# JJanai/back2future

Measured on AMD Instinct MI355X. Metric: frame-triplets/sec at 3x1024x1920, higher is better.
Workload: dtype f32; 1 GPU; BASELINE.json configs[4] per-GPU share: batch=16 synthetic 3x1024x1920 triplets per GPU, random-init pwc.lua weights (Ours-Hard shape), outputs flow + occ + est[3]; batch_per_gpu=16, global_batch=16, height=1024, width=1920, parallelism=dp1: independent triplets per rank, one RCCL weight broadcast at init, hip_graph=True

## Files before the change

### back2future_amd/csrc/b2f_api.hip

```cpp
#include "b2f_ctx.h"

#include <cmath>
#include <cstdio>
#include <cstdlib>

using namespace b2f;

static thread_local std::string g_err;
namespace b2f {
int api_fail(const std::string &m)
{
    g_err = m;
    return 1;
}
const std::string &api_error() { return g_err; }

ConvSeg cp8_seg(const float *ptr, int C, size_t hw)
{
    ConvSeg sgm;
    sgm.ptr = ptr;
    sgm.img_stride = (long)(hw * (size_t)((C + 7) / 8 * 8));
    sgm.chunk_stride = (long)(hw * 8);
    sgm.pix_stride = 8;
    sgm.nchunks = 0;
// ... 467 lines not shown
    const int head_id1 = find_conv(c, KIND_FEAT, 2, 2), head_id2 = find_conv(c, KIND_FEAT, 3, 1);
    const bool head_fused = c->bf16_direct >= 2 && P.h[2] >= 4 && P.w[2] >= 4 && head_id1 >= 0 && head_id2 >= 0 &&
                            c->packed[(size_t)head_id1].wino == 3 && c->packed[(size_t)head_id2].wino == 5;
    for (int l = 2; l <= 7; ++l) {
        const int hi = P.h[l - 1], wi = P.w[l - 1], ho = P.h[l], wo = P.w[l];
        const int Ci = (l == 2) ? kImgC : kFeat[l - 1], Co = kFeat[l];
        if (l == 2 && P.seq) {
            Scope sc(c, s, "conv_first_seq", cap);
            HIPCHK(launch_conv_first_seq(dev_in, in_kind, P.nimg, P.H, P.W, c->wpk_dev + c->first_w_off, c->wpk_dev + c->first_b_off,
                                         A + P.tmp, s));
        } else if (l == 2) {
            Scope sc(c, s, "conv_first", cap);
            HIPCHK(launch_conv_first((const float *)dev_in, unit, B, P.H, P.W, c->wpk_dev + c->first_w_off,
                                     c->wpk_dev + c->first_b_off, A + P.tmp, s));
        } else if (l == 3 && head_fused) {
            const ConvSeg in2f = cp8_seg(A + P.cs[2], Co, (size_t)ho * wo);
            CHK(run_conv(c, s, cap, find_conv(c, KIND_FEAT, l, 2), &in2f, P.nimg, ho, wo, 1, 1, A + P.cs[l]));
            continue;
        } else {
            const ConvSeg in1 = cp8_seg(A + P.cs[l - 1], Ci, (size_t)hi * wi);
            CHK(run_conv(c, s, cap, find_conv(c, KIND_FEAT, l, 1), &in1, P.nimg, hi, wi, 2, 1, A + P.tmp));
        }
        if (l == 2 && head_fused) {
            const PackedConv &p1 = c->packed[find_conv(c, KIND_FEAT, 2, 2)], &p2 = c->packed[find_conv(c, KIND_FEAT, 3, 1)];
            HeadLaunch hl;
            hl.in = A + P.tmp; hl.in_img_stride = (long)((size_t)ho * wo * 16); hl.in_chunk_stride = (long)((size_t)ho * wo * 8); hl.in_pix_stride = 8;
            hl.H1 = ho; hl.W1 = wo;
            hl.w1 = c->wpk_dev + p1.w_off; hl.b1 = c->wpk_dev + p1.b_off; hl.w2 = c->wpk_dev + p2.w_off; hl.b2 = c->wpk_dev + p2.b_off;
            hl.out = A + P.cs[2];
            hl.Ho = P.h[3]; hl.Wo = P.w[3]; hl.nimg = P.nimg;
            hl.out_img_stride = (long)((size_t)hl.Ho * hl.Wo * 32); hl.out_chunk_stride = (long)((size_t)hl.Ho * hl.Wo * 8); hl.out_pix_stride = 8;
            char hname[48];
            snprintf(hname, sizeof hname, c->profile_layers ? "convH16_16to32_%dx%d" : "conv_head16_bf16", ho, wo);
            Scope sc(c, s, hname, cap);
            HIPCHK(launch_conv_head16(hl, s));
            continue;
        }
        const ConvSeg in2 = cp8_seg(A + P.tmp, Co, (size_t)ho * wo);
        CHK(run_conv(c, s, cap, find_conv(c, KIND_FEAT, l, 2), &in2, P.nimg, ho, wo, 1, 1, A + P.cs[l]));
    }
    if (full) {
        Scope sc(c, s, "avgpool2", cap);
        const size_t img_f = (size_t)B * P.H * P.W * kImgC;
        for (int f = 0; f < 2; ++f) {
            const float *src = A + P.img + (size_t)(f == 0 ? 0 : 2) * img_f;
            for (int k = 2; k <= 5; ++k) {
                const int hk = P.H >> (k - 2), wk = P.W >> (k - 2);
                float *dst = A + P.ds[k] + (size_t)f * B * (hk / 2) * (wk / 2) * kImgC;
                HIPCHK(launch_avgpool2_nhwc(src, B, hk, wk, kImgC, dst, s));
                src = dst;
            }
        }
    }
    for (int l = 7; l >= 3; --l) {
        const int h = P.h[l], w = P.w[l], Cl = kFeat[l];
        const size_t hw = (size_t)h * w;
        CorrLaunch cl;
        cl.ref = A + P.cs[l] + (size_t)P.fo * hw * Cl;
        cl.nbr_fut = A + P.cs[l] + (size_t)2 * P.fo * hw * Cl;
        cl.nbr_past = A + P.cs[l];
        cl.img_stride = (long)(hw * Cl);
        cl.chunk_stride = (long)(hw * 8);
        cl.pix_stride = 8;
        cl.flow = (l < 7) ? A + P.U[l] : nullptr;
        cl.flow_b = (l < 7 && past) ? A + P.UB[l] : nullptr;
        cl.k = (float)(20.0 / std::pow(2.0, l - 1));
        cl.out = A + P.cv;
        cl.out_img_stride = (long)(hw * kCvRec);
        cl.out_chunk_stride = (long)(hw * 8);
        cl.out_pix_stride = 8;
        cl.B = B; cl.C = Cl; cl.h = h; cl.w = w;
        cl.variant = c->corr_variant;
        cl.ablate = c->corr_ablate;
        {
            char cname[48];
            snprintf(cname, sizeof cname, c->profile_layers ? "warp_costvol_%dx%d" : "warp_costvol", h, w);
            Scope sc(c, s, cname, cap);
            HIPCHK(launch_warp_costvol(cl, s));
        }
        float *occ_out = full ? O.t_occ[l] : (l == 3 ? O.occ : nullptr);
        float *occ_out2 = (!full && l == 3 && c->past_flow) ? O.est3 : nullptr;
        if (occ_out || occ_out2) {
            CHK(run_decoder(c, s, cap, P, KIND_OCC, l, A + P.logits));
            {
                Scope sc(c, s, "softmax_nearest4", cap);
                if (occ_out) HIPCHK(launch_softmax_nearest4_planar(A + P.logits, 8, B, h, w, occ_out, s));
                if (occ_out2) HIPCHK(launch_softmax_nearest4_planar(A + P.logits, 8, B, h, w, occ_out2, s));
            }
        }
        CHK(run_decoder(c, s, cap, P, KIND_FLOW, l, A + P.fs));
        if (past) CHK(run_decoder(c, s, cap, P, KIND_PAST, l, A + P.bfs));
        float *skip_f = full ? O.t_ufs[l] : (l == 3 ? (O.flow ? O.flow : A + P.flow_planar) : nullptr);
        {
            Scope sc(c, s, "upsample_flow2x", cap);
            float *u = (l > 3) ? A + P.U[l - 1] : A + P.u2;
            HIPCHK(launch_upsample_flow2x(A + P.fs, 8, B, h, w, u, s));
            if (skip_f) HIPCHK(launch_upsample_flow2x_planar(u, 2, B, 2 * h, 2 * w, skip_f, s));
            if (past) {
                float *ub = (l > 3) ? A + P.UB[l - 1] : A + P.d[1];
                HIPCHK(launch_upsample_flow2x(A + P.bfs, 8, B, h, w, ub, s));
                if (O.t_ubfs[l]) HIPCHK(launch_upsample_flow2x_planar(ub, 2, B, 2 * h, 2 * w, O.t_ubfs[l], s));
            }
        }
        if (full) {
            Scope sc(c, s, "warp_image", cap);
            const int k = l - 2;
            const int hk = 4 * h, wk = 4 * w;
            const size_t img_f = (size_t)B * hk * wk * kImgC;
            const float *im1 = (k == 1) ? A + P.img : A + P.ds[k];
            const float *im3 = (k == 1) ? A + P.img + 2 * img_f : A + P.ds[k] + img_f;
            const float kk = (float)(20.0 / std::pow(2.0, l - 3));
            const float *fl1 = (past && O.t_ubfs[l]) ? O.t_ubfs[l] : O.t_ufs[l];
            if (O.t_iw1[l]) HIPCHK(launch_warp_image_planar(im1, fl1, -kk, B, hk, wk, O.t_iw1[l], s));
            if (O.t_iw3[l]) HIPCHK(launch_warp_image_planar(im3, O.t_ufs[l], kk, B, hk, wk, O.t_iw3[l], s));
        }
    }
    if (!full && O.est3 && !c->past_flow && P.seq) {
        Scope sc(c, s, "warp_image_seq", cap);
        HIPCHK(launch_warp_input_seq(dev_in, in_kind, O.flow ? O.flow : A + P.flow_planar, -20.0f, B, P.H, P.W, O.est3, s));
    } else if (!full && O.est3 && !c->past_flow) {
        Scope sc(c, s, "warp_image", cap);
        HIPCHK(launch_warp_input_planar((const float *)dev_in, unit, 0, O.flow ? O.flow : A + P.flow_planar, -20.0f, B, P.H, P.W,
                                        O.est3, s));
    }
    return 0;
}

}
int b2f::find_conv_id(const b2f_ctx *c, int kind, int level, int idx) { return find_conv(c, kind, level, idx); }
int b2f::run_conv_layer(b2f_ctx *c, hipStream_t s, bool cap, int conv_id, const ConvSeg *segs, int nimg, int H, int W, int stride,
                        int leaky, float *out)
{
    if (conv_id < 0) return fail("b2f: layer not present in this model");
    return run_conv(c, s, cap, conv_id, segs, nimg, H, W, stride, leaky, out);
}
int b2f::ensure_arena(b2f_ctx *c, size_t floats) { return ensure_workspace_floats(c, floats); }
int b2f::check_shape(int B, int H, int W)
{
    if (B <= 0 || H <= 0 || W <= 0) return fail("b2f: non-positive shape");
    if (H % 64 || W % 64) return fail("b2f: H and W must be multiples of 64 (7 pyramid levels, back2future.lua:54-67)");
    return 0;
}
namespace {

bool parse_random(const char *name, bool *past, unsigned long long *seed, float *gain)
{
    if (strncmp(name, "random:", 7) != 0) return false;
    std::string s(name + 7);
    std::vector<std::string> parts;
    size_t pos = 0;
    while (true) {
        size_t q = s.find(':', pos);
        parts.push_back(s.substr(pos, q == std::string::npos ? q : q - pos));
        if (q == std::string::npos) break;
        pos = q + 1;
    }
    if (parts[0] == "hard") *past = false;
    else if (parts[0] == "soft") *past = true;
    else return false;
    *seed = 2;
    *gain = 1.f;
    if (parts.size() > 1 && !parts[1].empty()) *seed = strtoull(parts[1].c_str(), nullptr, 10);
    if (parts.size() > 2 && !parts[2].empty()) *gain = strtof(parts[2].c_str(), nullptr);
    return true;
}

bool ends_with(const std::string &s, const char *suf)
{
    const size_t n = strlen(suf);
// ... 106 lines not shown
        else if (path == "Ours-Soft-ft-KITTI") path = "models/RoamingImages_H_KITTI_S.t7";
        else if (path == "Ours-Soft-ft-Sintel") path = "models/RoamingImages_H_Sintel_S.t7";
        if (ends_with(path, ".t7")) {
            std::string err;
            if (!load_t7_ex(path, g, !(graph_opts && *graph_opts), flat, err)) return fail("b2f_init: " + err);
            past = g.past_flow;
        } else if (ends_with(path, ".b2fw")) {
            FILE *f = fopen(path.c_str(), "rb");
            if (!f) return fail("b2f_init: cannot open " + path);
            fseek(f, 0, SEEK_END);
            const long sz = ftell(f);
            fseek(f, 0, SEEK_SET);
            flat.resize((size_t)sz / 4);
            const size_t rd = fread(flat.data(), 4, flat.size(), f);
            fclose(f);
            if (rd != flat.size()) return fail("b2f_init: short read on " + path);
            GraphOpts gp = g, gn = g;
            gp.past_flow = true; gn.past_flow = false;
            if ((long long)flat.size() == param_count(gp)) past = true;
            else if ((long long)flat.size() == param_count(gn)) past = false;
            else return fail("b2f_init: " + path + " does not hold a parameter set of this graph (with or without past-flow decoders)");
        } else {
            return fail(std::string("b2f_init: unknown model '") + name + "'");
        }
    }
    b2f_ctx *c = new b2f_ctx();
    c->device = device;
    c->g = g;
    {
        auto env_int = [](const char *k, long long dflt) {
            const char *v = getenv(k);
            if (!v) return dflt;
            char *end = nullptr;
            const long long x = strtoll(v, &end, 10);
            return end == v ? 1ll : x;
        };
        c->wino4_min_pixels = (int)env_int("B2F_WINO4_MIN_PIXELS", c->wino4_min_pixels);
        c->wino_split_pixels = (int)env_int("B2F_WINO_SPLIT_PIXELS", c->wino_split_pixels);
        c->wino8 = (int)env_int("B2F_WINO8", c->wino8);
        c->adaptive_kernels = (int)env_int("B2F_ADAPTIVE_KERNELS", c->adaptive_kernels);
        c->corr_variant = (int)env_int("B2F_CORR_VARIANT", env_int("B2F_CORR_LAT", c->corr_variant));
        c->op_wino_split = (int)env_int("B2F_OP_WINO_SPLIT", c->op_wino_split);
        c->use_graph = (int)env_int("B2F_USE_GRAPH", c->use_graph);
        c->host_graph = (int)env_int("B2F_HOST_GRAPH", c->host_graph);
        c->profile = (int)env_int("B2F_PROFILE", c->profile);
        c->corr_ablate = (int)env_int("B2F_CORR_ABLATE", c->corr_ablate);
        c->profile_layers = (int)env_int("B2F_PROFILE_LAYERS", c->profile_layers);
        c->wino4_persistent = (int)env_int("B2F_WINO4_PERSISTENT", c->wino4_persistent);
        c->wino1d = (int)env_int("B2F_WINO1D", c->wino1d);
        c->wino6 = (int)env_int("B2F_WINO6", c->wino6);
        c->wino6_min_pixels = (int)env_int("B2F_WINO6_MIN_PIXELS", c->wino6_min_pixels);
        c->s2_loader = (int)env_int("B2F_S2_LOADER", c->s2_loader);
        c->s2_tile_groups = (int)env_int("B2F_S2_TILE_GROUPS", c->s2_tile_groups);
#if B2F_EXPERIMENTS
        c->wino4_split = (int)env_int("B2F_WINO4_SPLIT", c->wino4_split);
        c->wino4_hybrid = (int)env_int("B2F_WINO4_HYBRID", c->wino4_hybrid);
        c->wino2_split = (int)env_int("B2F_WINO2_SPLIT", c->wino2_split);
#endif
        if (!use_wino()) { c->bf16_conv = 0; c->bf16_direct = 0; }
        c->bf16_direct = (int)env_int("B2F_BF16_DIRECT", c->bf16_direct);
        c->bf16_conv = (int)env_int("B2F_BF16_CONV", c->bf16_conv);
        c->s2_tiles_per_block = (int)env_int("B2F_S2_TILES_PER_BLOCK", c->s2_tiles_per_block);
        c->host_subbatch_pixels = env_int("B2F_HOST_SUBBATCH_PIXELS", c->host_subbatch_pixels);
        c->host_threads = (int)env_int("B2F_HOST_THREADS", c->host_threads);
        c->host_u8 = (int)env_int("B2F_HOST_U8", c->host_u8);
        c->host_ramp = (int)env_int("B2F_HOST_RAMP", c->host_ramp);
#if !B2F_EXPERIMENTS
        if (c->corr_variant == 2 || c->corr_variant == 4 || c->corr_variant == 6 || c->corr_variant == 8) {
            fprintf(stderr, "b2f_init: B2F_CORR_VARIANT=%d is an experiment kernel (build with `python -m back2future_amd.build --experiments`): using the default\n", c->corr_variant);
            c->corr_variant = -1;
        }
        if (c->bf16_direct == 1) {
            fprintf(stderr, "b2f_init: B2F_BF16_DIRECT=1 is an experiment (build with `python -m back2future_amd.build --experiments`): using the default (2)\n");
            c->bf16_direct = 2;
        }
#endif
    }
    if (hipStreamCreateWithFlags(&c->stream, hipStreamDefault) != hipSuccess) {
        delete c;
        return fail("b2f_init: hipStreamCreate failed");
    }
    if (install_weights(c, flat.data(), (long long)flat.size(), past) != 0) {
        b2f_destroy(c);
        return 1;
    }
    *out = c;
    return 0;
}
B2F_CATCH("b2f_init_ex")

void b2f_destroy(b2f_ctx *c)
{
    if (!c) return;
    (void)hipSetDevice(c->device);
    if (c->stream) (void)hipStreamSynchronize(c->stream);
    drop_graphs(c);
    drop_gen_out(c);
    for (ProfEvent &pe : c->prof_pending) { (void)hipEventDestroy(pe.a); (void)hipEventDestroy(pe.b); }
    for (hipEvent_t e : c->ev_pool) (void)hipEventDestroy(e);
    for (HostSlot &hs : c->slot) {
        if (hs.dev) (void)hipFree(hs.dev);
        if (hs.pin) (void)hipHostFree(hs.pin);
        for (hipEvent_t e : {hs.ev_in, hs.ev_comp, hs.ev_out})
            if (e) (void)hipEventDestroy(e);
    }
    if (c->s_in) (void)hipStreamDestroy(c->s_in);
// ... 86 lines not shown
    }
    else if (!strcmp(key, "wino1d")) {
        HIPCHK(hipSetDevice(c->device));
        HIPCHK(hipDeviceSynchronize());
        drop_graphs(c);
        const bool had = c->wino1d != 0;
        c->wino1d = value;
        if (had != (value != 0)) CHK(b2f_commit_weights(c));
    }
    else if (!strcmp(key, "wino6") || !strcmp(key, "wino6_min_pixels")) {
        HIPCHK(hipSetDevice(c->device));
        HIPCHK(hipDeviceSynchronize());
        drop_graphs(c);
        if (key[5] == '_') c->wino6_min_pixels = value;
        else {
            const bool had = c->wino6 != 0;
            c->wino6 = value;
            if (had != (value != 0)) CHK(b2f_commit_weights(c));
        }
    }
#if !B2F_EXPERIMENTS
    else if (!strcmp(key, "wino2_split") || !strcmp(key, "wino4_split") || !strcmp(key, "wino4_hybrid")) {
        if (value != 0) return fail(std::string("b2f_set_option: ") + key + " selects an experiment kernel (tools/experiments/csrc): build with `python -m back2future_amd.build --experiments` and load libb2f_exp.so");
    }
#else
    else if (!strcmp(key, "wino2_split")) {
        HIPCHK(hipSetDevice(c->device));
        HIPCHK(hipDeviceSynchronize());
        drop_graphs(c);
        const bool had = c->wino2_split != 0;
        c->wino2_split = value;
        if (had != (value != 0)) CHK(b2f_commit_weights(c));
    }
    else if (!strcmp(key, "wino4_split") || !strcmp(key, "wino4_hybrid")) {
        HIPCHK(hipSetDevice(c->device));
        HIPCHK(hipDeviceSynchronize());
        drop_graphs(c);
        const bool had = c->wino4_split || c->wino4_hybrid;
        (key[6] == 's' ? c->wino4_split : c->wino4_hybrid) = value;
        if (had != (c->wino4_split || c->wino4_hybrid)) CHK(b2f_commit_weights(c));
    }
#endif
    else if (!strcmp(key, "s2_tiles_per_block") || !strcmp(key, "wino4_persistent")) {
        HIPCHK(hipSetDevice(c->device));
        HIPCHK(hipDeviceSynchronize());
        drop_graphs(c);
        (key[0] == 's' ? c->s2_tiles_per_block : c->wino4_persistent) = value;
    }
    else if (!strcmp(key, "s2_loader") || !strcmp(key, "s2_tile_groups")) {
        HIPCHK(hipSetDevice(c->device));
        HIPCHK(hipDeviceSynchronize());
        drop_graphs(c);
        (key[3] == 'l' ? c->s2_loader : c->s2_tile_groups) = value;
    }
    else if (!strcmp(key, "wino_split_pixels") || !strcmp(key, "wino8")) {
        HIPCHK(hipSetDevice(c->device));
        HIPCHK(hipDeviceSynchronize());
        drop_graphs(c);
        (key[4] == '8' ? c->wino8 : c->wino_split_pixels) = value;
    }
    else if (!strcmp(key, "wino4_min_pixels") || !strcmp(key, "adaptive_kernels")) {
        HIPCHK(hipSetDevice(c->device));
        HIPCHK(hipDeviceSynchronize());
        drop_graphs(c);
        (key[0] == 'w' ? c->wino4_min_pixels : c->adaptive_kernels) = value;
    } else if (!strcmp(key, "corr_variant") || !strcmp(key, "corr_ablate")) {
        HIPCHK(hipSetDevice(c->device));
        HIPCHK(hipDeviceSynchronize());
        drop_graphs(c);
        if (key[5] == 'v' && !B2F_EXPERIMENTS && (value == 2 || value == 4 || value == 6 || value == 8))
            return fail("b2f_set_option: corr_variant 2 / 4 / 6 / 8 are experiment kernels: build with `python -m back2future_amd.build --experiments`");
        (key[5] == 'v' ? c->corr_variant : c->corr_ablate) = value;
    } else if (!strcmp(key, "op_wino_split")) c->op_wino_split = value;
    else if (!strcmp(key, "host_subbatch_pixels")) c->host_subbatch_pixels = value > 0 ? value : (16ll << 20);
    else if (!strcmp(key, "host_threads")) c->host_threads = value;
    else if (!strcmp(key, "host_u8")) c->host_u8 = value;
    else if (!strcmp(key, "host_ramp")) c->host_ramp = value;
    else if (!strcmp(key, "debug_fail_next")) c->debug_fail_next = value;
    else return fail(std::string("b2f_set_option: unknown key ") + key);
    return 0;
}
B2F_CATCH("b2f_set_option")

int b2f_get_option(const b2f_ctx *c, const char *key, int *value) try
{
    if (!c || !key || !value) return fail("b2f_get_option: null argument");
    const std::string k(key);
    if (k == "use_graph") *value = c->use_graph;
    else if (k == "host_graph") *value = c->host_graph;
    else if (k == "profile") *value = c->profile;
    else if (k == "profile_layers") *value = c->profile_layers;
    else if (k == "s2_tiles_per_block") *value = c->s2_tiles_per_block;
    else if (k == "wino4_persistent") *value = c->wino4_persistent;
    else if (k == "experiments") *value = B2F_EXPERIMENTS;
    else if (k == "wino1d") *value = c->wino1d;
    else if (k == "wino6") *value = c->wino6;
    else if (k == "wino6_min_pixels") *value = c->wino6_min_pixels;
    else if (k == "s2_loader") *value = c->s2_loader;
    else if (k == "s2_tile_groups") *value = c->s2_tile_groups;
    else if (k == "wino4_split") *value = c->wino4_split;
    else if (k == "wino4_hybrid") *value = c->wino4_hybrid;
    else if (k == "wino2_split") *value = c->wino2_split;
    else if (k == "bf16_direct") *value = c->bf16_direct;
    else if (k == "bf16_conv") *value = c->bf16_conv;
    else if (k == "bf16_conv_min_pixels") *value = c->bf16_conv_min_pixels;
    else if (k == "wino4_min_pixels") *value = c->wino4_min_pixels;
    else if (k == "wino_split_pixels") *value = c->wino_split_pixels;
    else if (k == "wino8") *value = c->wino8;
    else if (k == "adaptive_kernels") *value = c->adaptive_kernels;
    else if (k == "corr_variant") *value = c->corr_variant;
    else if (k == "corr_ablate") *value = c->corr_ablate;
    else if (k == "op_wino_split") *value = c->op_wino_split;
    else if (k == "host_subbatch_pixels") *value = (int)std::min<long long>(c->host_subbatch_pixels, 0x7fffffff);
    else if (k == "host_threads") *value = c->host_threads;
    else if (k == "host_u8") *value = c->host_u8;
    else if (k == "host_ramp") *value = c->host_ramp;
    else if (k == "debug_fail_next") *value = c->debug_fail_next;
    else return fail("b2f_get_option: unknown key " + k);
    return 0;
}
B2F_CATCH("b2f_get_option")

int b2f_synchronize(b2f_ctx *c) try
{
    if (!c) return fail("b2f_synchronize: null context");
    HIPCHK(hipSetDevice(c->device));
    HIPCHK(hipStreamSynchronize(c->stream));
    return 0;
}
B2F_CATCH("b2f_synchronize")

int b2f_profile_reset(b2f_ctx *c) try
{
    if (!c) return fail("b2f_profile_reset: null context");
    CHK(prof_collect(c));
    std::fill(c->prof_ms.begin(), c->prof_ms.end(), 0.0);
    std::fill(c->prof_n.begin(), c->prof_n.end(), 0);
    return 0;
}
B2F_CATCH("b2f_profile_reset")

int b2f_profile_read(b2f_ctx *c, char *names, double *total_ms, long long *launches, int cap, int *n) try
{
    if (!c || !n) return fail("b2f_profile_read: null argument");
    CHK(prof_collect(c));
    const int cnt = std::min<int>(cap, (int)c->prof_names.size());
    for (int i = 0; i < cnt; ++i) {
        if (names) { strncpy(names + 32 * i, c->prof_names[i].c_str(), 31); names[32 * i + 31] = 0; }
        if (total_ms) total_ms[i] = c->prof_ms[i];
        if (launches) launches[i] = c->prof_n[i];
    }
    *n = cnt;
// ... 472 lines not shown
```

### back2future_amd/csrc/b2f_ctx.h

```cpp
#pragma once
#include "../../include/b2f.h"

#include <algorithm>
#include <atomic>
#include <condition_variable>
#include <cstring>
#include <exception>
#include <map>
#include <memory>
#include <mutex>
#include <string>
#include <thread>
#include <tuple>
#include <vector>

#include "b2f_host.h"
#include "b2f_internal.h"

namespace b2f {

int api_fail(const std::string &m);
const std::string &api_error();


// ... 189 lines not shown
            l.unlock();
            run_piece(j);
            l.lock();
            if (++done_ == pieces_->size()) cv_done_.notify_all();
        }
    }
    std::vector<std::thread> th_;
    std::mutex m_;
    std::condition_variable cv_, cv_done_;
    const std::vector<CopyJob> *pieces_ = nullptr;
    size_t next_ = 0, done_ = 0;
    bool stop_ = false;
};

}

struct b2f_ctx {
    int device = 0;
    bool past_flow = false;
    b2f::GraphOpts g;
    long long nparams = 0;
    hipStream_t stream = nullptr;
    std::vector<b2f::ConvDesc> lay;
    std::vector<b2f::PackedConv> packed;
    float *w_dev = nullptr;
    float *wpk_dev = nullptr;
    size_t wpk_floats = 0;
    size_t first_w_off = 0, first_b_off = 0;
    float *arena = nullptr;
    size_t arena_floats = 0;
    int wsB = 0, wsH = 0, wsW = 0;
    int use_graph = 0, profile = 0;
    int host_graph = 1;
    int wino8 = 1;
    int wino_split_pixels = 512;
    int wino4_min_pixels = 4096;
    int cur_batch = 0;
    int req_batch = 0;
    int adaptive_kernels = -1;
    int corr_ablate = 0;
    int corr_variant = -1;
    int op_wino_split = 0;
    int profile_layers = 0;
    int bf16_direct = 2;
    int bf16_conv_min_pixels = 65536;
    int bf16_conv = 1;
    int wino2_split = 0;
    int wino4_hybrid = 0;
    int wino4_split = 0;
    int wino6 = 1;
    int wino6_min_pixels = 16384;
    int wino1d = 0;
    int s2_tile_groups = 1;
    int s2_loader = 1;
    int wino4_persistent = 1;
    int s2_tiles_per_block = 0;
    long long host_subbatch_pixels = 16ll << 20;
    int host_threads = 0;
    int host_u8 = 1, host_ramp = 1;
    int debug_fail_next = 0;
    std::map<b2f::GraphKey, hipGraphExec_t> graphs;
    std::vector<float *> gen_out;
    int genB = 0, genH = 0, genW = 0;
    std::vector<std::string> prof_names;
    std::vector<double> prof_ms;
    std::vector<long long> prof_n;
    std::vector<b2f::ProfEvent> prof_pending;
    std::vector<hipEvent_t> ev_pool;
    hipStream_t s_in = nullptr, s_out = nullptr;
    b2f::HostSlot slot[2];
    std::unique_ptr<b2f::CopyPool> pool_in, pool_out;
    b2f::DevWork dwork;
};

#define HIPCHK(expr)                                                                         \
    do {                                                                                     \
        hipError_t e_ = (expr);                                                              \
        if (e_ != hipSuccess)                                                                \
            return b2f::api_fail(std::string(#expr) + ": " + hipGetErrorString(e_));          \
    } while (0)
#define B2F_CATCH(fn_)                                                                        \
    catch (const std::exception &e_) { return b2f::api_fail(std::string(fn_ ": ") + e_.what()); } \
    catch (...) { return b2f::api_fail(fn_ ": unknown exception"); }
#define CHK(expr)                         \
    do {                                  \
        int rc_ = (expr);                 \
        if (rc_ != 0) return rc_;         \
    } while (0)

namespace b2f {
int check_shape(int B, int H, int W);
void drop_graphs(b2f_ctx *c);
void drop_gen_out(b2f_ctx *c);
int forward_device(b2f_ctx *c, const void *dev_in, int in_kind, int B, int H, int W, float *dev_flow, float *dev_occ,
                   float *dev_est3, hipStream_t s, bool graph, bool seq = false);
int check_request(const FlowRequest &r);
int compute_flow_host(b2f_ctx *c, const FlowRequest &r);
int compute_flow_device(b2f_ctx *c, const FlowRequest &r, void *stream);
ConvSeg cp8_seg(const float *ptr, int C, size_t hw);
int find_conv_id(const b2f_ctx *c, int kind, int level, int idx);
int run_conv_layer(b2f_ctx *c, hipStream_t s, bool cap, int conv_id, const ConvSeg *segs, int nimg, int H, int W, int stride, int leaky,
                   float *out);
int ensure_arena(b2f_ctx *c, size_t floats);
int graph_forward(b2f_ctx *c, hipStream_t s, bool cap, const void *dev_in, int in_kind, int B, int H, int W, float *const *outs);
}
```

### back2future_amd/csrc/b2f_glue.hip

```cpp
#include "b2f_internal.h"

namespace b2f {

__global__ void pack_input_kernel(const float *in, int normalize, int B, int H, int W, float *img)
{
    const size_t hw = (size_t)H * W;
    const size_t i = (size_t)blockIdx.x * blockDim.x + threadIdx.x;
    if (i >= (size_t)B * hw) return;
    const size_t b = i / hw, p = i - b * hw;
#pragma unroll
    for (int f = 0; f < 3; ++f) {
        float v[3];
#pragma unroll
        for (int c = 0; c < 3; ++c) {
            float x = in[(b * 9 + f * 3 + c) * hw + p];
            if (normalize) x = color_normalize(x, c);
            v[c] = x;
        }
        float4 *o = reinterpret_cast<float4 *>(img + (((size_t)f * B + b) * hw + p) * kImgC);
        o[0] = make_float4(v[0], v[1], v[2], 0.f);
        o[1] = make_float4(0.f, 0.f, 0.f, 0.f);
    }
}

hipError_t launch_pack_input(const float *in, int normalize, int B, int H, int W, float *img, hipStream_t s)
{
    const size_t n = (size_t)B * H * W;
    hipLaunchKernelGGL(pack_input_kernel, dim3((unsigned)((n + 255) / 256)), dim3(256), 0, s, in, normalize, B, H, W, img);
    return hipGetLastError();
}


__global__ void warp_nhwc_kernel(const float *img, long img_stride, int pix_stride, int C, int ih, int iw,
                                 const float *grid, float k, int B, int gh, int gw, float *out,
                                 int out_pix_stride)
{
    const size_t total = (size_t)B * gh * gw * C;
    const size_t i = (size_t)blockIdx.x * blockDim.x + threadIdx.x;
    if (i >= total) return;
    const int c = (int)(i % C);
    size_t pix = i / C;
    const int x = (int)(pix % gw);
    const size_t row = pix / gw;
    const int y = (int)(row % gh);
    const int b = (int)(row / gh);
    const float2 g = *reinterpret_cast<const float2 *>(grid + pix * 2);
    int xl, yt;
    float wx, wy;
    bhwd_top_left(g.x * k + (float)x, iw, xl, wx);
    bhwd_top_left(g.y * k + (float)y, ih, yt, wy);
    const float *src = img + (size_t)b * img_stride + ((size_t)yt * iw + xl) * pix_stride + c;
    const bool x1 = xl + 1 <= iw - 1, y1 = yt + 1 <= ih - 1;
    const float tl = src[0];
    const float tr = x1 ? src[pix_stride] : 0.f;
    const float bl = y1 ? src[(size_t)iw * pix_stride] : 0.f;
    const float br = (x1 && y1) ? src[(size_t)(iw + 1) * pix_stride] : 0.f;
    out[pix * out_pix_stride + c] = wx * wy * tl + (1.f - wx) * wy * tr + wx * (1.f - wy) * bl + (1.f - wx) * (1.f - wy) * br;
}

hipError_t launch_warp_nhwc(const float *img, long img_stride, int pix_stride, int C, int ih, int iw,
                            const float *grid, float k, int B, int gh, int gw, float *out,
                            int out_pix_stride, hipStream_t s)
{
    const size_t n = (size_t)B * gh * gw * C;
    hipLaunchKernelGGL(warp_nhwc_kernel, dim3((unsigned)((n + 255) / 256)), dim3(256), 0, s, img, img_stride,
                       pix_stride, C, ih, iw, grid, k, B, gh, gw, out, out_pix_stride);
    return hipGetLastError();
}

__device__ __forceinline__ float2 bilerp2(const float *in, int ps, int h, int w, float rh, float rw, int y2, int x2)
{
    const float h1r = rh * (float)y2;
    const int h1 = (int)h1r;
    const int h1p = (h1 < h - 1) ? 1 : 0;
    const float h1l = h1r - (float)h1, h0l = 1.f - h1l;
    const float w1r = rw * (float)x2;
    const int w1 = (int)w1r;
    const int w1p = (w1 < w - 1) ? 1 : 0;
    const float w1l = w1r - (float)w1, w0l = 1.f - w1l;
    const float *p = in + ((size_t)h1 * w + w1) * ps;
    const float2 a = *reinterpret_cast<const float2 *>(p), b = *reinterpret_cast<const float2 *>(p + (size_t)w1p * ps);
    const float2 c = *reinterpret_cast<const float2 *>(p + (size_t)h1p * w * ps);
    const float2 d = *reinterpret_cast<const float2 *>(p + ((size_t)h1p * w + w1p) * ps);
    float2 o;
    o.x = h0l * (w0l * a.x + w1l * b.x) + h1l * (w0l * c.x + w1l * d.x);
    o.y = h0l * (w0l * a.y + w1l * b.y) + h1l * (w0l * c.y + w1l * d.y);
    return o;
}

__global__ __launch_bounds__(256) void upsample_flow2x_kernel(const float *in, int ps, int B, int h, int w, float *out, int planar)
{
    const int H2 = 2 * h, W2 = 2 * w;
    const int x0 = 4 * (int)(blockIdx.x * blockDim.x + threadIdx.x);
    const int y2 = (int)blockIdx.y, b = (int)blockIdx.z;
    if (x0 >= W2) return;
    const float rh = (H2 > 1) ? (float)(h - 1) / (float)(H2 - 1) : 0.f;
    const float rw = (W2 > 1) ? (float)(w - 1) / (float)(W2 - 1) : 0.f;
    const float *src = in + (size_t)b * h * w * ps;
    float2 o[4];
#pragma unroll
    for (int k = 0; k < 4; ++k) o[k] = bilerp2(src, ps, h, w, rh, rw, y2, min(x0 + k, W2 - 1));
    const size_t hw2 = (size_t)H2 * W2, row = (size_t)y2 * W2 + x0;
    if (planar) {
        float *o0 = out + ((size_t)b * 2) * hw2 + row, *o1 = o0 + hw2;
        if ((W2 & 3) == 0) {
            *reinterpret_cast<float4 *>(o0) = make_float4(o[0].x, o[1].x, o[2].x, o[3].x);
            *reinterpret_cast<float4 *>(o1) = make_float4(o[0].y, o[1].y, o[2].y, o[3].y);
        } else {
#pragma unroll
            for (int k = 0; k < 4; ++k)
                if (x0 + k < W2) { o0[k] = o[k].x; o1[k] = o[k].y; }
        }
    } else {
        float2 *op = reinterpret_cast<float2 *>(out) + (size_t)b * hw2 + row;
        if ((W2 & 3) == 0) {
            *reinterpret_cast<float4 *>(op) = make_float4(o[0].x, o[0].y, o[1].x, o[1].y);
            *reinterpret_cast<float4 *>(op + 2) = make_float4(o[2].x, o[2].y, o[3].x, o[3].y);
        } else {
#pragma unroll
            for (int k = 0; k < 4; ++k)
                if (x0 + k < W2) op[k] = o[k];
        }
    }
}

static hipError_t launch_upsample(const float *in, int in_pix_stride, int B, int h, int w, float *out, int planar, hipStream_t s)
{
    if (B <= 0 || h <= 0 || w <= 0) return hipSuccess;
    if (2 * h > 65535 || B > 65535) return hipErrorInvalidValue;
    const int groups = (2 * w + 3) / 4;
    hipLaunchKernelGGL(upsample_flow2x_kernel, dim3((unsigned)((groups + 255) / 256), (unsigned)(2 * h), (unsigned)B), dim3(256), 0, s, in,
                       in_pix_stride, B, h, w, out, planar);
    return hipGetLastError();
}
hipError_t launch_upsample_flow2x(const float *in, int in_pix_stride, int B, int h, int w, float *out, hipStream_t s)
{
    return launch_upsample(in, in_pix_stride, B, h, w, out, 0, s);
}
hipError_t launch_upsample_flow2x_planar(const float *in, int in_pix_stride, int B, int h, int w, float *out, hipStream_t s)
{
    return launch_upsample(in, in_pix_stride, B, h, w, out, 1, s);
}

__global__ __launch_bounds__(256) void softmax_nearest4_kernel(const float *logits, int ps, int B, int h, int w, float *out)
{
    const int H4 = 4 * h, W4 = 4 * w;
    const int x = (int)(blockIdx.x * blockDim.x + threadIdx.x);
    const int Y = (int)blockIdx.y, b = (int)blockIdx.z;
    if (x >= w) return;
    const float2 z = *reinterpret_cast<const float2 *>(logits + (((size_t)b * h + (Y >> 2)) * w + x) * ps);
    const float m = fmaxf(z.x, z.y);
    const float e0 = expf(z.x - m), e1 = expf(z.y - m);
    const float sum = e0 + e1;
    const float p0 = e0 / sum, p1 = e1 / sum;
    const size_t hw4 = (size_t)H4 * W4;
    float *o0 = out + ((size_t)b * 2) * hw4 + (size_t)Y * W4 + 4 * x;
    *reinterpret_cast<float4 *>(o0) = make_float4(p0, p0, p0, p0);
    *reinterpret_cast<float4 *>(o0 + hw4) = make_float4(p1, p1, p1, p1);
}

hipError_t launch_softmax_nearest4_planar(const float *logits, int in_pix_stride, int B, int h, int w, float *out, hipStream_t s)
{
    if (B <= 0 || h <= 0 || w <= 0) return hipSuccess;
    if (4 * h > 65535 || B > 65535) return hipErrorInvalidValue;
    hipLaunchKernelGGL(softmax_nearest4_kernel, dim3((unsigned)((w + 255) / 256), (unsigned)(4 * h), (unsigned)B), dim3(256), 0, s, logits,
                       in_pix_stride, B, h, w, out);
    return hipGetLastError();
}

__global__ void warp_image_planar_kernel(const float *img8, const float *flow, float k, int B, int H, int W, float *out)
{
    const size_t hw = (size_t)H * W;
    const size_t i = (size_t)blockIdx.x * blockDim.x + threadIdx.x;
    if (i >= (size_t)B * hw) return;
    const size_t b = i / hw, p = i - b * hw;
    const int y = (int)(p / W), x = (int)(p - (size_t)y * W);
    const float u = flow[(b * 2) * hw + p] * k, v = flow[(b * 2 + 1) * hw + p] * k;
    int xl, yt;
    float wx, wy;
    bhwd_top_left(u + (float)x, W, xl, wx);
    bhwd_top_left(v + (float)y, H, yt, wy);
    const float *src = img8 + (b * hw + (size_t)yt * W + xl) * kImgC;
    const bool x1 = xl + 1 <= W - 1, y1 = yt + 1 <= H - 1;
    const float4 z = make_float4(0.f, 0.f, 0.f, 0.f);
    const float4 tl = *reinterpret_cast<const float4 *>(src);
    const float4 tr = x1 ? *reinterpret_cast<const float4 *>(src + kImgC) : z;
    const float4 bl = y1 ? *reinterpret_cast<const float4 *>(src + (size_t)W * kImgC) : z;
    const float4 br = (x1 && y1) ? *reinterpret_cast<const float4 *>(src + (size_t)(W + 1) * kImgC) : z;
    const float w00 = wx * wy, w01 = (1.f - wx) * wy, w10 = wx * (1.f - wy), w11 = (1.f - wx) * (1.f - wy);
    out[(b * 3) * hw + p] = w00 * tl.x + w01 * tr.x + w10 * bl.x + w11 * br.x;
    out[(b * 3 + 1) * hw + p] = w00 * tl.y + w01 * tr.y + w10 * bl.y + w11 * br.y;
    out[(b * 3 + 2) * hw + p] = w00 * tl.z + w01 * tr.z + w10 * bl.z + w11 * br.z;
}

hipError_t launch_warp_image_planar(const float *img8, const float *flow_planar, float k, int B, int H, int W,
                                    float *out, hipStream_t s)
{
    const size_t n = (size_t)B * H * W;
    hipLaunchKernelGGL(warp_image_planar_kernel, dim3((unsigned)((n + 255) / 256)), dim3(256), 0, s, img8, flow_planar, k, B, H, W, out);
    return hipGetLastError();
}


__global__ __launch_bounds__(256) __attribute__((amdgpu_waves_per_eu(8, 8))) void conv_first_kernel(const float *in, int normalize, int B, int H, int W,
                                                         const float *wt , const float *bias ,
                                                         float *out )
{
// ... 140 lines not shown
                    const int pp = (ty + ky) * P + tx + kx;
                    const float4 lo = patch[c][0][pp], hi = patch[c][1][pp];
                    const float4 *wk = wsh + (c * 9 + ky * 3 + kx) * 4;
                    const float4 w0 = wk[0], w1 = wk[1], w2 = wk[2], w3 = wk[3];
                    a0 = fmaf(lo.x, w0.x, a0);  a1 = fmaf(lo.x, w0.y, a1);
                    a0 = fmaf(lo.y, w0.z, a0);  a1 = fmaf(lo.y, w0.w, a1);
                    a0 = fmaf(lo.z, w1.x, a0);  a1 = fmaf(lo.z, w1.y, a1);
                    a0 = fmaf(lo.w, w1.z, a0);  a1 = fmaf(lo.w, w1.w, a1);
                    a0 = fmaf(hi.x, w2.x, a0);  a1 = fmaf(hi.x, w2.y, a1);
                    a0 = fmaf(hi.y, w2.z, a0);  a1 = fmaf(hi.y, w2.w, a1);
                    a0 = fmaf(hi.z, w3.x, a0);  a1 = fmaf(hi.z, w3.y, a1);
                    a0 = fmaf(hi.w, w3.z, a0);  a1 = fmaf(hi.w, w3.w, a1);
                }
        }
    }
    const int oy = oy0 + ty, ox = ox0 + tx;
    if (oy >= H || ox >= W) return;
    if (leaky) { a0 = a0 > 0.f ? a0 : 0.2f * a0; a1 = a1 > 0.f ? a1 : 0.2f * a1; }
    float *op = out + (size_t)img * out_img_stride + ((size_t)oy * W + ox) * out_pix_stride;
    *reinterpret_cast<float2 *>(op) = make_float2(a0, a1);
}

hipError_t launch_conv_narrow2(const ConvLaunch &p, hipStream_t s)
{
    if (p.stride != 1 || p.cout != 2 || p.nseg != 1 || (p.seg[0].pix_stride & 3) || (p.out_pix_stride & 1)) return hipErrorInvalidValue;
    const int tiles = ((p.W + 15) / 16) * ((p.H + 15) / 16);
    if ((long)tiles * p.nimg <= 3L * device_cu_count() && p.seg[0].nchunks > 2)
        hipLaunchKernelGGL(conv_narrow2_kernel<4>, dim3((unsigned)(tiles * p.nimg)), dim3(256), 0, s, p.seg[0].ptr, p.seg[0].img_stride,
                           p.seg[0].chunk_stride, p.seg[0].pix_stride, p.seg[0].nchunks, p.H, p.W, p.wpk, p.bias, p.out,
                           p.out_img_stride, p.out_pix_stride, p.leaky);
    else
        hipLaunchKernelGGL(conv_narrow2_kernel<2>, dim3((unsigned)(tiles * p.nimg)), dim3(256), 0, s, p.seg[0].ptr, p.seg[0].img_stride,
                           p.seg[0].chunk_stride, p.seg[0].pix_stride, p.seg[0].nchunks, p.H, p.W, p.wpk, p.bias, p.out,
                           p.out_img_stride, p.out_pix_stride, p.leaky);
    return hipGetLastError();
}

size_t narrow2_wpk_floats(int cin_chunks) { return (size_t)cin_chunks * 9 * 8 * 2; }

void narrow2_pack_weights(const float *w, const float *b, int Ci, const int *cin_map, int cin_chunks, float *wpk, float *bpk)
{
    for (int c = 0; c < cin_chunks; ++c)
        for (int t = 0; t < 9; ++t)
            for (int j = 0; j < 8; ++j)
                for (int o = 0; o < 2; ++o) {
                    const int k = c * kCK + j;
                    const int ci = cin_map ? cin_map[k] : (k < Ci ? k : -1);
                    wpk[((c * 9 + t) * 8 + j) * 2 + o] = ci >= 0 ? w[((size_t)o * Ci + ci) * 9 + t] : 0.f;
                }
    bpk[0] = b[0];
    bpk[1] = b[1];
}

__global__ void warp_input_planar_kernel(const float *in, int normalize, int frame, const float *flow, float k, int B,
                                         int H, int W, float *out)
{
    const size_t hw = (size_t)H * W;
    const size_t i = (size_t)blockIdx.x * blockDim.x + threadIdx.x;
    if (i >= (size_t)B * hw) return;
    const size_t b = i / hw, p = i - b * hw;
    const int y = (int)(p / W), x = (int)(p - (size_t)y * W);
    const float u = flow[(b * 2) * hw + p] * k, v = flow[(b * 2 + 1) * hw + p] * k;
    int xl, yt;
    float wx, wy;
    bhwd_top_left(u + (float)x, W, xl, wx);
    bhwd_top_left(v + (float)y, H, yt, wy);
    const int dx = (xl + 1 <= W - 1) ? 1 : 0, dy = (yt + 1 <= H - 1) ? W : 0;
    const float w00 = wx * wy, w01 = (1.f - wx) * wy, w10 = wx * (1.f - wy), w11 = (1.f - wx) * (1.f - wy);
#pragma unroll
    for (int c = 0; c < 3; ++c) {
        const float *src = in + (b * 9 + (size_t)frame * 3 + c) * hw + (size_t)yt * W + xl;
        float tl = src[0], tr = src[dx], bl = src[dy], br = src[dy + dx];
        if (normalize) {
            tl = color_normalize(tl, c); tr = color_normalize(tr, c);
            bl = color_normalize(bl, c); br = color_normalize(br, c);
        }
        out[(b * 3 + c) * hw + p] = w00 * tl + w01 * tr + w10 * bl + w11 * br;
    }
}

hipError_t launch_warp_input_planar(const float *in, int normalize, int frame, const float *flow_planar, float k, int B,
                                    int H, int W, float *out, hipStream_t s)
{
    const size_t n = (size_t)B * H * W;
    hipLaunchKernelGGL(warp_input_planar_kernel, dim3((unsigned)((n + 255) / 256)), dim3(256), 0, s, in, normalize, frame,
                       flow_planar, k, B, H, W, out);
    return hipGetLastError();
}

__global__ void avgpool2_kernel(const float *in, int nimg, int H, int W, int C, float *out)
{
    const int Ho = H / 2, Wo = W / 2, C4 = C / 4;
    const size_t n = (size_t)nimg * Ho * Wo * C4;
    const size_t i = (size_t)blockIdx.x * blockDim.x + threadIdx.x;
    if (i >= n) return;
    const int c4 = (int)(i % C4);
    size_t pix = i / C4;
    const int X = (int)(pix % Wo);
    const size_t r = pix / Wo;
    const int Y = (int)(r % Ho);
    const size_t b = r / Ho;
    const float4 *s = reinterpret_cast<const float4 *>(in) + ((b * H + 2 * Y) * W + 2 * X) * C4 + c4;
    const float4 a = s[0], bb = s[C4], c = s[(size_t)W * C4], d = s[(size_t)(W + 1) * C4];
    float4 o;
    o.x = (a.x + bb.x + c.x + d.x) / 4.0f;
    o.y = (a.y + bb.y + c.y + d.y) / 4.0f;
    o.z = (a.z + bb.z + c.z + d.z) / 4.0f;
    o.w = (a.w + bb.w + c.w + d.w) / 4.0f;
    reinterpret_cast<float4 *>(out)[i] = o;
}

hipError_t launch_avgpool2_nhwc(const float *in, int nimg, int H, int W, int C, float *out, hipStream_t s)
{
    const size_t n = (size_t)nimg * (H / 2) * (W / 2) * (C / 4);
    hipLaunchKernelGGL(avgpool2_kernel, dim3((unsigned)((n + 255) / 256)), dim3(256), 0, s, in, nimg, H, W, C, out);
    return hipGetLastError();
}

__global__ void nhwc_to_planar_kernel(const float *in, int pix_stride, int C, int B, int h, int w, float *out)
{
    const size_t hw = (size_t)h * w;
    const size_t n = (size_t)B * C * hw;
    const size_t i = (size_t)blockIdx.x * blockDim.x + threadIdx.x;
    if (i >= n) return;
    const size_t p = i % hw;
    const size_t bc = i / hw;
    const int c = (int)(bc % C);
    const size_t b = bc / C;
    out[i] = in[(b * hw + p) * pix_stride + c];
}

hipError_t launch_nhwc_to_planar(const float *in, int pix_stride, int C, int B, int h, int w, float *out, hipStream_t s)
{
    const size_t n = (size_t)B * C * h * w;
    hipLaunchKernelGGL(nhwc_to_planar_kernel, dim3((unsigned)((n + 255) / 256)), dim3(256), 0, s, in, pix_stride, C, B, h, w, out);
    return hipGetLastError();
}

__global__ void cp8_to_planar_kernel(const float *in, int C, int B, int h, int w, float *out)
// ... 54 lines not shown
```

### back2future_amd/csrc/b2f_internal.h

```cpp
#pragma once
#include <hip/hip_runtime.h>
#ifndef B2F_EXPERIMENTS
#define B2F_EXPERIMENTS 0
#endif
#include <cstdint>

namespace b2f {

constexpr int kLevels = 7, kLst = 3, kWin = 9, kND = 2 * kWin * kWin;
constexpr int kFeat[8] = {0, 3, 16, 32, 64, 96, 128, 192};
constexpr int kDec[7] = {0, 128, 128, 96, 64, 32, 2};
constexpr int kCvRec = 168;
constexpr int kCvChunks = 21;
constexpr int kImgC = 8;
constexpr int kCK = 8;

struct ConvSeg {
    const float *ptr;
    long img_stride;
    long chunk_stride;
    int pix_stride;
    int nchunks;
};
struct ConvLaunch {
// ... 130 lines not shown
    int ablate = 0;
    int variant = -1;
};
inline int attr_slot()
{
    int dev = 0;
    if (hipGetDevice(&dev) != hipSuccess || dev < 0) dev = 0;
    return dev & 63;
}
inline int device_cu_count()
{
    static int n_cu_dev[64] = {0};
    int &n = n_cu_dev[attr_slot()];
    if (!n) {
        int dev = 0, v = 0;
        if (hipGetDevice(&dev) != hipSuccess || hipDeviceGetAttribute(&v, hipDeviceAttributeMultiprocessorCount, dev) != hipSuccess || v <= 0) v = 256;
        n = v < 8 ? 8 : v;
    }
    return n;
}
#ifdef __HIPCC__
__device__ __forceinline__ int xcd_remap(int bid, int nwg)
{
    const int q = nwg >> 3, r = nwg & 7;
    const int xcd = bid & 7, k = bid >> 3;
    return (xcd < r ? xcd * (q + 1) : r * (q + 1) + (xcd - r) * q) + k;
}
__device__ __forceinline__ void bhwd_top_left(float coord, int size, int &pt, float &wt)
{
    float c = coord;
    if (c < 0.f) c = 0.f;
    if (c > (float)(size - 1)) c = (float)(size - 1);
    const float fl = floorf(c);
    pt = (int)fl;
    wt = 1.f - (c - fl);
}
#endif

inline int cv_slot(int dir, int c) { return c < 80 ? dir * 80 + c : 160 + dir; }
hipError_t launch_warp_costvol(const CorrLaunch &p, hipStream_t s);
bool warp_costvol_unit_supported(const CorrLaunch &p);
hipError_t launch_warp_costvol_unit(const CorrLaunch &p, hipStream_t s);
hipError_t launch_warp_costvol_spec(const CorrLaunch &p, hipStream_t s);
hipError_t launch_warp_costvol_gw(const CorrLaunch &p, hipStream_t s);
hipError_t launch_costvol_generic(const float *ref, const float *frm, int B, int C, int h, int w,
                                  int win, int fwd, float *out, hipStream_t s);

hipError_t launch_pack_input(const float *in, int normalize, int B, int H, int W, float *img,
                             hipStream_t s);
hipError_t launch_conv_first(const float *in, int normalize, int B, int H, int W, const float *wt,
                             const float *bias, float *out, hipStream_t s);
hipError_t launch_warp_input_planar(const float *in, int normalize, int frame, const float *flow_planar,
                                    float k, int B, int H, int W, float *out, hipStream_t s);
hipError_t launch_conv_first_seq(const void *in, int in_kind, int T, int H, int W, const float *wt, const float *bias,
                                 float *out, hipStream_t s);
hipError_t launch_warp_input_seq(const void *in, int in_kind, const float *flow_planar, float k, int B, int H, int W,
                                 float *out, hipStream_t s);
hipError_t launch_warp_nhwc(const float *img, long img_stride, int pix_stride, int C, int ih,
                            int iw, const float *grid, float k, int B, int gh, int gw,
                            float *out, int out_pix_stride, hipStream_t s);
hipError_t launch_upsample_flow2x(const float *in, int in_pix_stride, int B, int h, int w, float *out,
                                  hipStream_t s);
hipError_t launch_upsample_flow2x_planar(const float *in, int in_pix_stride, int B, int h, int w,
                                         float *out, hipStream_t s);
hipError_t launch_softmax_nearest4_planar(const float *logits, int in_pix_stride, int B, int h, int w,
                                          float *out, hipStream_t s);
hipError_t launch_warp_image_planar(const float *img8, const float *flow_planar, float k, int B,
                                    int H, int W, float *out, hipStream_t s);
hipError_t launch_avgpool2_nhwc(const float *in, int nimg, int H, int W, int C, float *out,
                                hipStream_t s);
hipError_t launch_nhwc_to_planar(const float *in, int pix_stride, int C, int B, int h, int w,
                                 float *out, hipStream_t s);
hipError_t launch_cp8_to_planar(const float *in, int C, int B, int h, int w, float *out, hipStream_t s);
hipError_t launch_planar_to_nhwc(const float *in, int C, int B, int h, int w, float *out,
                                 int pix_stride, hipStream_t s);
hipError_t launch_fill(float *p, size_t n, float v, hipStream_t s);

hipError_t launch_image_scale(const float *src, int normalize, long planes, int Hs, int Ws, float *tmp, float *dst,
                              int Hd, int Wd, hipStream_t s);
hipError_t launch_outputs_f32(const float *flow_net, const float *occ, const float *est3, int est3_ch, int B, int fh, int fw, int H0,
                              int W0, double sc_w, double sc_h, float *flow, float *occ_prob, unsigned char *fwd_occ,
                              unsigned char *bwd_occ, hipStream_t s);
hipError_t launch_unpack_u8(const unsigned char *in, size_t n, float *out, hipStream_t s);

}
```

Measured before the change: 845.1 triplets/s.

## Fuse final flow upsampling, occlusion softmax and input warp into one kernel

```diff
diff --git a/back2future_amd/csrc/b2f_api.hip b/back2future_amd/csrc/b2f_api.hip
--- a/back2future_amd/csrc/b2f_api.hip
+++ b/back2future_amd/csrc/b2f_api.hip
@@ -543,6 +543,7 @@
             }
         }
     }
+    const bool fused_out = c->output_fused && !full && !c->past_flow && !P.seq && O.est3 && in_kind != B2F_IN_U8 && P.H == 4 * P.h[3] && P.W == 4 * P.w[3];
     for (int l = 7; l >= 3; --l) {
         const int h = P.h[l], w = P.w[l], Cl = kFeat[l];
         const size_t hw = (size_t)h * w;
@@ -569,11 +570,12 @@
             Scope sc(c, s, cname, cap);
             HIPCHK(launch_warp_costvol(cl, s));
         }
+        const bool out_fused = l == 3 && fused_out;
         float *occ_out = full ? O.t_occ[l] : (l == 3 ? O.occ : nullptr);
         float *occ_out2 = (!full && l == 3 && c->past_flow) ? O.est3 : nullptr;
         if (occ_out || occ_out2) {
             CHK(run_decoder(c, s, cap, P, KIND_OCC, l, A + P.logits));
-            {
+            if (!out_fused) {
                 Scope sc(c, s, "softmax_nearest4", cap);
                 if (occ_out) HIPCHK(launch_softmax_nearest4_planar(A + P.logits, 8, B, h, w, occ_out, s));
                 if (occ_out2) HIPCHK(launch_softmax_nearest4_planar(A + P.logits, 8, B, h, w, occ_out2, s));
@@ -581,6 +583,12 @@
         }
         CHK(run_decoder(c, s, cap, P, KIND_FLOW, l, A + P.fs));
         if (past) CHK(run_decoder(c, s, cap, P, KIND_PAST, l, A + P.bfs));
+        if (out_fused) {
+            Scope sc(c, s, "flow_output", cap);
+            HIPCHK(launch_flow_output(A + P.fs, O.occ ? A + P.logits : nullptr, 8, (const float *)dev_in, unit, -20.0f, B, h, w,
+                                      O.flow ? O.flow : A + P.flow_planar, O.occ, O.est3, s));
+            continue;
+        }
         float *skip_f = full ? O.t_ufs[l] : (l == 3 ? (O.flow ? O.flow : A + P.flow_planar) : nullptr);
         {
             Scope sc(c, s, "upsample_flow2x", cap);
@@ -606,6 +614,7 @@
             if (O.t_iw3[l]) HIPCHK(launch_warp_image_planar(im3, O.t_ufs[l], kk, B, hk, wk, O.t_iw3[l], s));
         }
     }
+    if (fused_out) return 0;
     if (!full && O.est3 && !c->past_flow && P.seq) {
         Scope sc(c, s, "warp_image_seq", cap);
         HIPCHK(launch_warp_input_seq(dev_in, in_kind, O.flow ? O.flow : A + P.flow_planar, -20.0f, B, P.H, P.W, O.est3, s));
@@ -818,6 +827,7 @@
         c->wino6_min_pixels = (int)env_int("B2F_WINO6_MIN_PIXELS", c->wino6_min_pixels);
         c->s2_loader = (int)env_int("B2F_S2_LOADER", c->s2_loader);
         c->s2_tile_groups = (int)env_int("B2F_S2_TILE_GROUPS", c->s2_tile_groups);
+        c->output_fused = (int)env_int("B2F_OUTPUT_FUSED", c->output_fused);
 #if B2F_EXPERIMENTS
         c->wino4_split = (int)env_int("B2F_WINO4_SPLIT", c->wino4_split);
         c->wino4_hybrid = (int)env_int("B2F_WINO4_HYBRID", c->wino4_hybrid);
@@ -1010,6 +1020,12 @@
         HIPCHK(hipDeviceSynchronize());
         drop_graphs(c);
         (key[3] == 'l' ? c->s2_loader : c->s2_tile_groups) = value;
+    }
+    else if (!strcmp(key, "output_fused")) {
+        HIPCHK(hipSetDevice(c->device));
+        HIPCHK(hipDeviceSynchronize());
+        drop_graphs(c);
+        c->output_fused = value;
     }
     else if (!strcmp(key, "wino_split_pixels") || !strcmp(key, "wino8")) {
         HIPCHK(hipSetDevice(c->device));
@@ -1056,6 +1072,7 @@
     else if (k == "wino6_min_pixels") *value = c->wino6_min_pixels;
     else if (k == "s2_loader") *value = c->s2_loader;
     else if (k == "s2_tile_groups") *value = c->s2_tile_groups;
+    else if (k == "output_fused") *value = c->output_fused;
     else if (k == "wino4_split") *value = c->wino4_split;
     else if (k == "wino4_hybrid") *value = c->wino4_hybrid;
     else if (k == "wino2_split") *value = c->wino2_split;
diff --git a/back2future_amd/csrc/b2f_ctx.h b/back2future_amd/csrc/b2f_ctx.h
--- a/back2future_amd/csrc/b2f_ctx.h
+++ b/back2future_amd/csrc/b2f_ctx.h
@@ -265,6 +265,7 @@
     int wino6_min_pixels = 16384;
     int wino1d = 0;
     int s2_tile_groups = 1;
+    int output_fused = 1;
     int s2_loader = 1;
     int wino4_persistent = 1;
     int s2_tiles_per_block = 0;
diff --git a/back2future_amd/csrc/b2f_glue.hip b/back2future_amd/csrc/b2f_glue.hip
--- a/back2future_amd/csrc/b2f_glue.hip
+++ b/back2future_amd/csrc/b2f_glue.hip
@@ -68,24 +68,29 @@
     return hipGetLastError();
 }
 
+struct Lerp1 { int i, p; float l1, l0; };
+__device__ __forceinline__ Lerp1 lerp_axis(float r, int o, int n)
+{
+    const float f = r * (float)o;
+    const int i = (int)f;
+    const float l1 = f - (float)i;
+    return Lerp1{i, (i < n - 1) ? 1 : 0, l1, 1.f - l1};
+}
+__device__ __forceinline__ float2 bilerp2_mix(const Lerp1 &hy, const Lerp1 &wx, float2 a, float2 b, float2 c, float2 d)
+{
+    float2 o;
+    o.x = hy.l0 * (wx.l0 * a.x + wx.l1 * b.x) + hy.l1 * (wx.l0 * c.x + wx.l1 * d.x);
+    o.y = hy.l0 * (wx.l0 * a.y + wx.l1 * b.y) + hy.l1 * (wx.l0 * c.y + wx.l1 * d.y);
+    return o;
+}
 __device__ __forceinline__ float2 bilerp2(const float *in, int ps, int h, int w, float rh, float rw, int y2, int x2)
 {
-    const float h1r = rh * (float)y2;
-    const int h1 = (int)h1r;
-    const int h1p = (h1 < h - 1) ? 1 : 0;
-    const float h1l = h1r - (float)h1, h0l = 1.f - h1l;
-    const float w1r = rw * (float)x2;
-    const int w1 = (int)w1r;
-    const int w1p = (w1 < w - 1) ? 1 : 0;
-    const float w1l = w1r - (float)w1, w0l = 1.f - w1l;
-    const float *p = in + ((size_t)h1 * w + w1) * ps;
-    const float2 a = *reinterpret_cast<const float2 *>(p), b = *reinterpret_cast<const float2 *>(p + (size_t)w1p * ps);
-    const float2 c = *reinterpret_cast<const float2 *>(p + (size_t)h1p * w * ps);
-    const float2 d = *reinterpret_cast<const float2 *>(p + ((size_t)h1p * w + w1p) * ps);
-    float2 o;
-    o.x = h0l * (w0l * a.x + w1l * b.x) + h1l * (w0l * c.x + w1l * d.x);
-    o.y = h0l * (w0l * a.y + w1l * b.y) + h1l * (w0l * c.y + w1l * d.y);
-    return o;
+    const Lerp1 hy = lerp_axis(rh, y2, h), wx = lerp_axis(rw, x2, w);
+    const float *p = in + ((size_t)hy.i * w + wx.i) * ps;
+    const float2 a = *reinterpret_cast<const float2 *>(p), b = *reinterpret_cast<const float2 *>(p + (size_t)wx.p * ps);
+    const float2 c = *reinterpret_cast<const float2 *>(p + (size_t)hy.p * w * ps);
+    const float2 d = *reinterpret_cast<const float2 *>(p + ((size_t)hy.p * w + wx.p) * ps);
+    return bilerp2_mix(hy, wx, a, b, c, d);
 }
 
 __global__ __launch_bounds__(256) void upsample_flow2x_kernel(const float *in, int ps, int B, int h, int w, float *out, int planar)
@@ -142,6 +147,13 @@
     return launch_upsample(in, in_pix_stride, B, h, w, out, 1, s);
 }
 
+__device__ __forceinline__ float2 softmax2(const float2 z)
+{
+    const float m = fmaxf(z.x, z.y);
+    const float e0 = expf(z.x - m), e1 = expf(z.y - m);
+    const float sum = e0 + e1;
+    return make_float2(e0 / sum, e1 / sum);
+}
 __global__ __launch_bounds__(256) void softmax_nearest4_kernel(const float *logits, int ps, int B, int h, int w, float *out)
 {
     const int H4 = 4 * h, W4 = 4 * w;
@@ -149,10 +161,8 @@
     const int Y = (int)blockIdx.y, b = (int)blockIdx.z;
     if (x >= w) return;
     const float2 z = *reinterpret_cast<const float2 *>(logits + (((size_t)b * h + (Y >> 2)) * w + x) * ps);
-    const float m = fmaxf(z.x, z.y);
-    const float e0 = expf(z.x - m), e1 = expf(z.y - m);
-    const float sum = e0 + e1;
-    const float p0 = e0 / sum, p1 = e1 / sum;
+    const float2 pr = softmax2(z);
+    const float p0 = pr.x, p1 = pr.y;
     const size_t hw4 = (size_t)H4 * W4;
     float *o0 = out + ((size_t)b * 2) * hw4 + (size_t)Y * W4 + 4 * x;
     *reinterpret_cast<float4 *>(o0) = make_float4(p0, p0, p0, p0);
@@ -399,15 +409,10 @@
     bpk[1] = b[1];
 }
 
-__global__ void warp_input_planar_kernel(const float *in, int normalize, int frame, const float *flow, float k, int B,
-                                         int H, int W, float *out)
-{
-    const size_t hw = (size_t)H * W;
-    const size_t i = (size_t)blockIdx.x * blockDim.x + threadIdx.x;
-    if (i >= (size_t)B * hw) return;
-    const size_t b = i / hw, p = i - b * hw;
-    const int y = (int)(p / W), x = (int)(p - (size_t)y * W);
-    const float u = flow[(b * 2) * hw + p] * k, v = flow[(b * 2 + 1) * hw + p] * k;
+__device__ __forceinline__ void warp_input_pixel(const float *in, int normalize, int frame, size_t b, size_t hw, int H, int W, int x, int y,
+                                                 float fu, float fv, float k, float o[3])
+{
+    const float u = fu * k, v = fv * k;
     int xl, yt;
     float wx, wy;
     bhwd_top_left(u + (float)x, W, xl, wx);
@@ -422,8 +427,21 @@
             tl = color_normalize(tl, c); tr = color_normalize(tr, c);
             bl = color_normalize(bl, c); br = color_normalize(br, c);
         }
-        out[(b * 3 + c) * hw + p] = w00 * tl + w01 * tr + w10 * bl + w11 * br;
-    }
+        o[c] = w00 * tl + w01 * tr + w10 * bl + w11 * br;
+    }
+}
+__global__ void warp_input_planar_kernel(const float *in, int normalize, int frame, const float *flow, float k, int B,
+                                         int H, int W, float *out)
+{
+    const size_t hw = (size_t)H * W;
+    const size_t i = (size_t)blockIdx.x * blockDim.x + threadIdx.x;
+    if (i >= (size_t)B * hw) return;
+    const size_t b = i / hw, p = i - b * hw;
+    const int y = (int)(p / W), x = (int)(p - (size_t)y * W);
+    float o[3];
+    warp_input_pixel(in, normalize, frame, b, hw, H, W, x, y, flow[(b * 2) * hw + p], flow[(b * 2 + 1) * hw + p], k, o);
+#pragma unroll
+    for (int c = 0; c < 3; ++c) out[(b * 3 + c) * hw + p] = o[c];
 }
 
 hipError_t launch_warp_input_planar(const float *in, int normalize, int frame, const float *flow_planar, float k, int B,
@@ -432,6 +450,82 @@
     const size_t n = (size_t)B * H * W;
     hipLaunchKernelGGL(warp_input_planar_kernel, dim3((unsigned)((n + 255) / 256)), dim3(256), 0, s, in, normalize, frame,
                        flow_planar, k, B, H, W, out);
+    return hipGetLastError();
+}
+
+namespace flow_out {
+constexpr int TH = 8, TW = 128, NR = 6, NC = 66;
+}
+__global__ __launch_bounds__(256) void flow_output_kernel(const float *fs, const float *logits, int ps, const float *in, int normalize,
+                                                          float k, int h, int w, float *flow, float *occ, float *est3)
+{
+    using namespace flow_out;
+    __shared__ float2 u2[NR * NC];
+    __shared__ float fl[2][TH * TW];
+    const int h2 = 2 * h, w2 = 2 * w, H = 4 * h, W = 4 * w;
+    const size_t hw = (size_t)H * W;
+    const int b = (int)blockIdx.z, Y0 = TH * (int)blockIdx.y, X0 = TW * (int)blockIdx.x;
+    const int tid = (int)threadIdx.x;
+    const float rh1 = (h2 > 1) ? (float)(h - 1) / (float)(h2 - 1) : 0.f, rw1 = (w2 > 1) ? (float)(w - 1) / (float)(w2 - 1) : 0.f;
+    const float rh2 = (H > 1) ? (float)(h2 - 1) / (float)(H - 1) : 0.f, rw2 = (W > 1) ? (float)(w2 - 1) / (float)(W - 1) : 0.f;
+    const int r_lo = lerp_axis(rh2, Y0, h2).i, c_lo = lerp_axis(rw2, X0, w2).i;
+    {
+        const float *src = fs + (size_t)b * h * w * ps;
+        for (int e = tid; e < NR * NC; e += 256) {
+            const int r = e / NC, cc = e - r * NC;
+            u2[e] = bilerp2(src, ps, h, w, rh1, rw1, min(r_lo + r, h2 - 1), min(c_lo + cc, w2 - 1));
+        }
+    }
+    __syncthreads();
+    {
+        const int row = tid >> 5, X = X0 + 4 * (tid & 31), Y = Y0 + row;
+        if (X < W) {
+            const Lerp1 hy = lerp_axis(rh2, Y, h2);
+            const int ra = min(hy.i - r_lo, NR - 1) * NC, rb = min(hy.i + hy.p - r_lo, NR - 1) * NC;
+            float2 o[4];
+#pragma unroll
+            for (int q = 0; q < 4; ++q) {
+                const Lerp1 wx = lerp_axis(rw2, X + q, w2);
+                const int ca = min(wx.i - c_lo, NC - 1), cb = min(wx.i + wx.p - c_lo, NC - 1);
+                o[q] = bilerp2_mix(hy, wx, u2[ra + ca], u2[ra + cb], u2[rb + ca], u2[rb + cb]);
+            }
+            const float4 ox = make_float4(o[0].x, o[1].x, o[2].x, o[3].x), oy = make_float4(o[0].y, o[1].y, o[2].y, o[3].y);
+            const size_t p4 = (size_t)Y * W + X;
+            float *f0 = flow + ((size_t)b * 2) * hw + p4;
+            *reinterpret_cast<float4 *>(f0) = ox;
+            *reinterpret_cast<float4 *>(f0 + hw) = oy;
+            *reinterpret_cast<float4 *>(&fl[0][row * TW + 4 * (tid & 31)]) = ox;
+            *reinterpret_cast<float4 *>(&fl[1][row * TW + 4 * (tid & 31)]) = oy;
+            if (occ) {
+                const float2 pr = softmax2(*reinterpret_cast<const float2 *>(logits + (((size_t)b * h + (Y >> 2)) * w + (X >> 2)) * ps));
+                float *o0 = occ + ((size_t)b * 2) * hw + p4;
+                *reinterpret_cast<float4 *>(o0) = make_float4(pr.x, pr.x, pr.x, pr.x);
+                *reinterpret_cast<float4 *>(o0 + hw) = make_float4(pr.y, pr.y, pr.y, pr.y);
+            }
+        }
+    }
+    __syncthreads();
+#pragma unroll
+    for (int q = 0; q < 4; ++q) {
+        const int t = tid + 256 * q;
+        const int y = Y0 + (t >> 7), x = X0 + (t & (TW - 1));
+        if (x >= W) continue;
+        float e[3];
+        warp_input_pixel(in, normalize, 0, (size_t)b, hw, H, W, x, y, fl[0][t], fl[1][t], k, e);
+        const size_t p = (size_t)y * W + x;
+#pragma unroll
+        for (int c = 0; c < 3; ++c) est3[((size_t)b * 3 + c) * hw + p] = e[c];
+    }
+}
+
+hipError_t launch_flow_output(const float *fs, const float *logits, int in_pix_stride, const float *in, int normalize, float k, int B,
+                              int h, int w, float *flow, float *occ, float *est3, hipStream_t s)
+{
+    using namespace flow_out;
+    if (B <= 0 || h <= 0 || w <= 0) return hipSuccess;
+    if ((4 * h) % TH || 4 * h / TH > 65535 || B > 65535 || (in_pix_stride & 1) || (occ && !logits)) return hipErrorInvalidValue;
+    hipLaunchKernelGGL(flow_output_kernel, dim3((unsigned)((4 * w + TW - 1) / TW), (unsigned)(4 * h / TH), (unsigned)B), dim3(256), 0, s, fs,
+                       logits, in_pix_stride, in, normalize, k, h, w, flow, occ, est3);
     return hipGetLastError();
 }
 
diff --git a/back2future_amd/csrc/b2f_internal.h b/back2future_amd/csrc/b2f_internal.h
--- a/back2future_amd/csrc/b2f_internal.h
+++ b/back2future_amd/csrc/b2f_internal.h
@@ -206,6 +206,8 @@
                              const float *bias, float *out, hipStream_t s);
 hipError_t launch_warp_input_planar(const float *in, int normalize, int frame, const float *flow_planar,
                                     float k, int B, int H, int W, float *out, hipStream_t s);
+hipError_t launch_flow_output(const float *fs, const float *logits, int in_pix_stride, const float *in, int normalize, float k, int B,
+                              int h, int w, float *flow, float *occ, float *est3, hipStream_t s);
 hipError_t launch_conv_first_seq(const void *in, int in_kind, int T, int H, int W, const float *wt, const float *bias,
                                  float *out, hipStream_t s);
 hipError_t launch_warp_input_seq(const void *in, int in_kind, const float *flow_planar, float k, int B, int H, int W,
```

After: 844.3 triplets/s, median of 2. No clear change (-0.1%).
